# Nicholasli1995/SNVC

Measured on AMD Instinct MI355X. Metric: stereo-pairs/sec (cost-volume build + 3D CNN fwd), higher is better.
Workload: dtype f32 (split f16x3 operands, fp32 accumulate)

## Files before the change

snvc_amd/csrc/conv3d_f16.hip:

```cpp
#include <type_traits>

#include "common.hpp"
#include "elementwise_internal.hpp"
#include "snvc_fused.h"

namespace snvc {
namespace {

typedef _Float16 h8 __attribute__((ext_vector_type(8)));
typedef float f32x16 __attribute__((ext_vector_type(16)));
typedef float f32x4 __attribute__((ext_vector_type(4)));

__device__ const unsigned g_zero16h[4] __attribute__((aligned(16))) = {0u, 0u, 0u, 0u};

struct F16Args {
    const _Float16 *x;
    const _Float16 *wp;
    const float *scale, *bias;
    const _Float16 *res;
    _Float16 *y;
    float *y_f32;
    const _Float16 *x_lo, *res_lo;
    _Float16 *y_lo;
    const float *head;
    float *y_head;
    float head_mul;
    float res_mul;
    int *overflow;
    const _Float16 *tail_w;
    float *t_out;
    float tail_mul;
    int64_t t_bs;
    const float *res_f32;
    double *stats;
    const float *x_mul;
    int CGin;
    int Cout;
    int Din, Hin, Win;
    int Dout, Hout, Wout;
    int nd, nh, nw;
    int osd, osh, osw, offd, offh, offw;
    int pad_d, pad_h, pad_w;
    int isd, ish, iod, ioh;
    int tiles_d, tiles_h, tiles_w;
    int nchunks, flags;
    int N, cls_mode;
    int64_t cls_wstride;
    int64_t x_bs, y_bs, r_bs, yf_bs;
};

template <class I>
__host__ __device__ __forceinline__ I il_index(int mode, I oc, I C, I H, I pitch, I lp, I cls0, I h, I x) {
    const I cls = mode ? oc % 3 : oc / C, co = mode ? oc / 3 : oc % C, groups = (C + 7) / 8;
    return ((((cls0 + cls) * groups + (co >> 3)) * H + h) * pitch + lp + x) * 8 + (co & 7);
}

struct F16IlArgs : F16Args {
    float *y_il;
    int64_t il_bs;
    int il_mode, il_C, il_pitch, il_lp, il_cls0;
};

struct F16SrcArgs : F16Args {
    const float *gi;
    const float *p_il;
    const float *v_scale, *v_bias;
    int64_t gi_bs;
    int v_pitch, v_lp, v_q, v_m0, v_off, v_off2, v_flags;
};


template <int KD_, int KH_, int KW_, int STRIDE_, int DIL_, int MI_, int TD_, int TH_, int KCG_, int MODE_, bool DB_, int OCC_,
          int DILW_ = DIL_, int PL_ = 1, bool DYN_ = false>
struct F16Cfg {
    static constexpr bool DYN = DYN_;
    static constexpr int PL = PL_;
    static constexpr bool SPLIT = PL_ >= 2, SERIAL = PL_ == 3;
    static constexpr int RES_PL = PL_ == 2 ? 2 : 1;
    static constexpr int PASSES = SERIAL ? 2 : 1;
    static constexpr int PF = DYN_ ? 2 : (SPLIT ? 3 : 6);
    static constexpr int KD = KD_, KH = KH_, KW = KW_, STRIDE = STRIDE_, DIL = DIL_, DILW = DILW_, MI = MI_, TD = TD_, TH = TH_;
    static constexpr int KCG = KCG_, MODE = MODE_, OCC = OCC_;
    static constexpr bool DB = DB_;
    static constexpr int IN_D = (TD - 1) * STRIDE + (KD - 1) * DIL + 1;
    static constexpr int IN_H = (TH - 1) * STRIDE + (KH - 1) * DIL + 1;
    static constexpr int IN_W = 31 * STRIDE + (KW - 1) * DILW + 1;
    static constexpr int VOX = IN_D * IN_H * IN_W;
    static constexpr int GB = VOX * 16;
    static constexpr int ITEMS = RES_PL * KCG * VOX;
    static constexpr int PLANE_BYTES = KCG * GB;
    static constexpr int NIT = (ITEMS + 255) / 256;
    static constexpr int IMG_BYTES = NIT * 256 * 16;
    static constexpr int LDS_BYTES = IMG_BYTES * (DB ? 2 : 1);
    static constexpr int NB = TD * TH / 4;
    static constexpr bool UNROLL_D = KD <= 3;
    static constexpr int SEGS = UNROLL_D ? 1 : KD;
    static constexpr int TSEG = UNROLL_D ? KD * KH * KW : KH * KW;
    static constexpr int NPS = (TSEG + 1) / 2;
    static constexpr int NS = MODE == 0 ? TSEG * (KCG / 2) : NPS * KCG;
    static constexpr int STEPS = SEGS * NS;
    static constexpr int SEG_BYTES = DIL * IN_H * IN_W * 16;
    static_assert(TD * TH % 4 == 0, "rows split over 4 waves");
// ... 520 lines not shown
__device__ __forceinline__ void lds_read_b128_to(h8 &v, unsigned addr) {
    asm volatile("ds_read_b128 %0, %1 offset:%2" : "=v"(v) : "v"(addr), "n"(IMM) : "memory");
}

template <int N>
__device__ __forceinline__ void wait_lgkm_for(h8 (&b)[8]) {
    asm volatile("s_waitcnt lgkmcnt(%8)"
                 : "+v"(b[0]), "+v"(b[1]), "+v"(b[2]), "+v"(b[3]), "+v"(b[4]), "+v"(b[5]), "+v"(b[6]), "+v"(b[7])
                 : "n"(N)
                 : "memory");
}

template <int SRC, class A>
__device__ __forceinline__ const F16SrcArgs &src_args_of(const A &a) {
    if constexpr (SRC == 1) return a;
    else return *reinterpret_cast<const F16SrcArgs *>(&a);
}

template <int EPI, int SRC = 0>
__global__ void __launch_bounds__(256, 2)
conv3d_x3q_kernel(const std::conditional_t<SRC == 1, F16SrcArgs, F16Args> a) {
    using Cfg = X3QCfg;
    constexpr int NB = Cfg::NB, TH = Cfg::TH, IN_H = Cfg::IN_H, IN_W = Cfg::IN_W, VOX = Cfg::VOX, NIT = Cfg::NIT, NQ = Cfg::NQ;
    constexpr int ITEMS = Cfg::ITEMS, PF = Cfg::PF;
    extern __shared__ __attribute__((aligned(16))) char lds[];
    const int tid = threadIdx.x, lane = tid & 63, wave = tid >> 6, kb = lane >> 4, col = lane & 15;
    const int ntiles = a.tiles_d * a.tiles_h * a.tiles_w, cblocks = a.Cout >> 5;
    const int job = xcd_remap16(blockIdx.x, ntiles * cblocks);
    const int t = job / cblocks, cb = job - t * cblocks;
    const int tw = t % a.tiles_w, th = (t / a.tiles_w) % a.tiles_h, td = t / (a.tiles_w * a.tiles_h);
    const int64_t n = blockIdx.z;
    const int od0 = td * Cfg::TD, oh0 = th * TH, ow0 = tw * 32;
    const int id0 = od0 - a.pad_d, ih0 = oh0 - a.pad_h, iw0 = ow0 - a.pad_w;

    f32x4q acc[NB][2][2];
#pragma unroll
    for (int nb = 0; nb < NB; ++nb)
#pragma unroll
        for (int ph = 0; ph < 2; ++ph)
#pragma unroll
            for (int h = 0; h < 2; ++h) acc[nb][ph][h] = f32x4q{0.0f, 0.0f, 0.0f, 0.0f};

    const int in_hw = a.Hin * a.Win, in_dhw = in_hw * a.Din;
    unsigned off[NIT];
    unsigned vmask = 0, pmask = 0;
#pragma unroll
    for (int it = 0; it < NIT; ++it) {
        const int i = it * 256 + tid;
        const int plane = i / VOX, r = i - plane * VOX;
        pmask |= (unsigned)(plane & 1) << it;
        const int dd = r / (IN_H * IN_W), r2 = r - dd * (IN_H * IN_W);
        const int hh = r2 / IN_W, ww = r2 - hh * IN_W;
        const int gd = id0 + dd, gh = ih0 + hh, gw = iw0 + ww;
        const bool ok = i < ITEMS && (unsigned)gd < (unsigned)a.Din && (unsigned)gh < (unsigned)a.Hin && (unsigned)gw < (unsigned)a.Win;
        off[it] = ok ? (unsigned)(gd * in_hw + gh * a.Win + gw) : 0u;
        vmask |= (ok ? 1u : 0u) << it;
    }
    const _Float16 *xn = a.x + n * a.x_bs, *xn_lo = a.x_lo + n * a.x_bs;
    const int wbase = tid & ~63;
    auto issue = [&](int chunk, int buf) {
        const int64_t coff = (int64_t)chunk * in_dhw * 8;
        char *const ibuf = lds + buf * Cfg::IMG_BYTES;
#pragma unroll
        for (int it = 0; it < NIT; ++it) {
            const _Float16 *xc = (((pmask >> it) & 1u) ? xn_lo : xn) + coff;
            const void *src = ((vmask >> it) & 1u) ? static_cast<const void *>(xc + (size_t)off[it] * 8) : static_cast<const void *>(g_zero16h);
// ... 287 lines not shown
    for (int nb = 0; nb < NB; ++nb) {
        const int row = wave * NB + nb;
        const int pd = od0 + row / TH, phh = oh0 + row % TH;
#pragma unroll
        for (int ph = 0; ph < 2; ++ph) {
            const int pw = ow0 + 16 * ph + col;
            const bool ok = pd < a.nd && phh < a.nh && pw < a.nw;
            const int64_t sp = ok ? ((int64_t)pd * out_hw + phh * a.Wout + pw) : 0;
            h8 o, ol;
            float hsum = 0.0f;
#pragma unroll
            for (int e = 0; e < 8; ++e) {
                float v = __builtin_fmaf(acc[nb][ph][e >> 2][e & 3], sc[e], bi[e]);
                v = __builtin_amdgcn_fmed3f(v, lo_bound, kHalfMax);
                vmax = __builtin_fmaxf(vmax, ok ? __builtin_fabsf(v) : 0.0f);
                if constexpr (EPI == 3) hsum += hw8[e] * v;
                o[e] = (_Float16)v;
                ol[e] = (_Float16)(v - (float)o[e]);
            }
            if (ok) {
                *reinterpret_cast<h8 *>(yn + sp * 8) = o;
                *reinterpret_cast<h8 *>(yn_lo + sp * 8) = ol;
            }
            if constexpr (EPI == 3) {
                float tot = hsum + __shfl_xor(hsum, 16, 64);
                tot += __shfl_xor(tot, 32, 64);
                if (ok && kb == 0) a.y_head[n * out_dhw + sp] = tot * a.head_mul;
            }
        }
    }
    if (vmax >= kHalfMax && a.overflow) atomicOr(a.overflow, 1);
}

template <int KH_, int KW_>
struct X2QCfg {
    static constexpr int KH = KH_, KW = KW_, TH = 16, NB = 4, IN_H = TH + KH - 1, IN_W = 32 + KW - 1, VOX = IN_H * IN_W, GB = VOX * 16;
    static constexpr int ITEMS = 2 * VOX, PLANE_BYTES = GB, NIT = (ITEMS + 255) / 256;
    static constexpr int IMG_BYTES = NIT * 256 * 16, LDS_BYTES = 2 * IMG_BYTES;
    static constexpr int TAPS = KH * KW, NQ = (TAPS + 3) / 4, PF = 2, FILL_STEP = NQ - PF;
    static_assert(NQ > PF, "the refill is issued PF k-steps before the chunk ends");
};

template <class Cfg, int IL = 0>
__global__ void __launch_bounds__(256, 2)
conv2d_x3q_kernel(const std::conditional_t<IL == 1, F16IlArgs, F16Args> a) {
    constexpr int NB = Cfg::NB, IN_W = Cfg::IN_W, VOX = Cfg::VOX, NIT = Cfg::NIT, NQ = Cfg::NQ;
    constexpr int ITEMS = Cfg::ITEMS, PF = Cfg::PF;
    extern __shared__ __attribute__((aligned(16))) char lds[];
    const int tid = threadIdx.x, lane = tid & 63, wave = tid >> 6, kb = lane >> 4, col = lane & 15;
    const int ntiles = a.tiles_h * a.tiles_w, cblocks = a.Cout >> 5;
    const int job = xcd_remap16(blockIdx.x, ntiles * cblocks);
    const int t = job / cblocks, cb = job - t * cblocks;
    const int tw = t % a.tiles_w, th = t / a.tiles_w;
    const int64_t n = blockIdx.z;
    const int oh0 = th * Cfg::TH, ow0 = tw * 32;
    const int ih0 = oh0 - a.pad_h, iw0 = ow0 - a.pad_w;

    f32x4q acc[NB][2][2];
#pragma unroll
    for (int nb = 0; nb < NB; ++nb)
#pragma unroll
        for (int ph = 0; ph < 2; ++ph)
#pragma unroll
            for (int h = 0; h < 2; ++h) acc[nb][ph][h] = f32x4q{0.0f, 0.0f, 0.0f, 0.0f};

    const int in_hw = a.Hin * a.Win;
// ... 863 lines not shown

struct Q16Layout { int K3, NSEG, NQ, NH, NPL, PASSES; };

struct F16Form {
    PackArgs pack;
    Q16Layout q16;
    int MI, KCG;
    int chunk_frags;
    int pad_frags;
    int cls_mode, TD, TH, grid;
    bool split_res, stats;
    const char *unsupported;
    F16Launch launch[F16_CALLS];

    constexpr F16Form on(F16Call c, F16Launch l) const { F16Form f = *this; f.launch[c] = l; return f; }
};

template <class Cfg, int EPI>
void launch_f16(const F16Args &a, const F16Geom &g, hipStream_t st) {
    launch_lds<conv3d_f16_kernel<Cfg, EPI>>(g.grid, 256, Cfg::LDS_BYTES, st, a);
}
template <class Cfg>
void launch_q16s(const F16Args &a, const F16Geom &g, hipStream_t st) {
    launch_lds<conv3d_q16s_kernel<Cfg>>(g.grid, 256, Cfg::LDS_BYTES, st, a);
}
template <int EPI>
void launch_x3q(const F16Args &a, const F16Geom &g, hipStream_t st) {
    launch_lds<conv3d_x3q_kernel<EPI>>(g.grid, 256, X3QCfg::LDS_BYTES, st, a);
}
template <int EPI>
void launch_x3q_src(const F16Args &a, const F16Geom &g, hipStream_t st) {
    launch_lds<conv3d_x3q_kernel<EPI, 1>>(g.grid, 256, X3QCfg::LDS_BYTES, st, static_cast<const F16SrcArgs &>(a));
}
void launch_x3s2q(const F16Args &a, const F16Geom &g, hipStream_t st) {
    int wg = device_cu_count();
    if (wg <= 0) wg = 256;
    if (g.jobs < wg) wg = g.jobs >= 8 ? (int)(g.jobs & ~(int64_t)7) : (int)g.jobs;
    launch_lds<conv3d_x3s2q_kernel>(dim3((unsigned)wg), X3S2Cfg::THREADS, X3S2Cfg::LDS_BYTES, st, a, (int)g.jobs);
}

template <class Cfg, int... EPI>
constexpr F16Form f16_form(int cls_mode, bool stats = false) {
    constexpr F16Call call_of[5] = {TO_C8, TO_PLANE, TO_F32, TO_HEAD, TO_TAIL};
    constexpr int npl = Cfg::PL >= 2 ? 2 : 1;
    F16Form f{};
    f.pack.KD = Cfg::KD; f.pack.KH = Cfg::KH; f.pack.KW = Cfg::KW; f.pack.KCG = Cfg::KCG; f.pack.MODE = Cfg::MODE; f.pack.MI = Cfg::MI;
    f.pack.SEGS = Cfg::SEGS; f.pack.TSEG = Cfg::TSEG; f.pack.NPS = Cfg::NPS; f.pack.NS = Cfg::NS; f.pack.unroll_d = Cfg::UNROLL_D ? 1 : 0;
    f.pack.PL = Cfg::PL; f.pack.PASSES = Cfg::PASSES; f.pack.dyn = Cfg::DYN ? 1 : 0;
    f.MI = Cfg::MI; f.KCG = Cfg::KCG; f.TD = Cfg::TD; f.TH = Cfg::TH;
    f.chunk_frags = Cfg::PASSES * Cfg::STEPS * Cfg::MI * npl;
    f.pad_frags = Cfg::PF * Cfg::MI * npl;
    f.cls_mode = cls_mode; f.grid = GRID_TILES; f.split_res = true; f.stats = stats;
    f.unsupported = Cfg::PL >= 2 ? "snvc_f16x3_conv3d_forward: no kernel" : "snvc_f16_conv3d_forward: no kernel";
    ((f.launch[call_of[EPI]] = launch_f16<Cfg, EPI>), ...);
    return f;
}

constexpr F16Form q16_form(Q16Layout q, int TD, int TH, int pad_steps, int cls_mode, int grid, bool split_res, bool stats, const char *unsupported) {
    F16Form f{};
    f.q16 = q; f.MI = q.NH / 2; f.KCG = 1; f.TD = TD; f.TH = TH;
    f.chunk_frags = q.PASSES * q.NSEG * q.NQ * q.NH * q.NPL;
    f.pad_frags = pad_steps * q.NH * q.NPL;
    f.cls_mode = cls_mode; f.grid = grid; f.split_res = split_res; f.stats = stats; f.unsupported = unsupported;
    return f;
}
template <class C>
// ... 367 lines not shown
    a.res_f32 = c.res_f32;
    a.stats = c.stats;
    a.x_mul = to_f32 ? c.x_mul : nullptr;
    a.tail_w = reinterpret_cast<const _Float16 *>(c.tail_w); a.t_out = c.t_out; a.tail_mul = c.tail_mul;
    a.t_bs = (int64_t)27 * 8 * d->Din * d->Hin * d->Win;
    a.CGin = d->Cin / 8; a.Cout = d->Cout;
    a.Din = d->Din; a.Hin = d->Hin; a.Win = d->Win;
    a.Dout = d->Dout; a.Hout = d->Hout; a.Wout = d->Wout;
    a.nchunks = p.nchunks; a.flags = flags;
    a.x_bs = d->x_batch_stride ? d->x_batch_stride : 2 * (int64_t)d->Cin * in_sp;
    a.y_bs = d->y_batch_stride ? d->y_batch_stride : 2 * (int64_t)d->Cout * out_sp;
    a.r_bs = d->res_batch_stride ? d->res_batch_stride : 2 * (int64_t)d->Cout * out_sp;
    a.yf_bs = plane ? out_sp : (d->y_batch_stride ? d->y_batch_stride : (int64_t)d->Cout * out_sp);
    const F16Geom g = f16_geometry(*d, p, a);
    if (g.ntiles >= ((int64_t)1 << 30) || (int64_t)d->N * g.classes > 65535)
        return fail(SNVC_ERR_UNSUPPORTED, "snvc_f16x3_conv3d_forward: too many tiles or samples");
    hipStream_t st = as_stream(c.stream);
    if (c.stats_slots) {
        if (!(to_f32 && !plane && !tail && f.stats))
            return fail(SNVC_ERR_UNSUPPORTED, "snvc_f16x3_conv3d_forward_stats: this layer's kernel form has no statistics epilogue");
        *c.stats_slots = g.stats_slots;
        if (!c.stats) return fail(SNVC_ERR_INVALID_ARGUMENT, "snvc_f16x3_conv3d_forward_stats: null workspace");
        if (g.classes > 1) {
            const hipError_t e = hipMemsetAsync(c.stats, 0, (size_t)d->N * g.stats_slots * ((d->Cout + 31) / 32) * 64 * sizeof(double), st);
            if (e != hipSuccess) return fail(SNVC_ERR_HIP, "snvc_f16x3_conv3d_forward_stats: hipMemsetAsync failed");
        }
    }
    if (c.src && !f.launch[TO_SRC])
        return fail(SNVC_ERR_UNSUPPORTED, "snvc_fused_first_conv3d_forward: a 3x3x3 stride-1 layer on the 16x16x32 form (SNVC_ALGO_X3_Q16)");
    const F16Call call = tail ? TO_TAIL : plane ? TO_PLANE : to_f32 ? TO_F32 : c.head ? (c.src ? TO_SRC_HEAD : TO_HEAD) : (c.src ? TO_SRC : TO_C8);
    if (!f.launch[call] || (resflags && !f.split_res)) return fail(SNVC_ERR_UNSUPPORTED, f.unsupported);
    if (g.jobs >= ((int64_t)1 << 30)) return fail(SNVC_ERR_UNSUPPORTED, "snvc_f16x3_conv3d_forward: too many tiles");
    if (c.src && to_f32) return fail(SNVC_ERR_UNSUPPORTED, "snvc_fused_first_conv3d_forward: a split C8 output");
    f.launch[call](b, g, st);
    return check_launch("snvc_f16x3_conv3d_forward");
}

int snvc_f16x3_conv3d_forward(const snvc_conv3d_desc *d, const void *x_hi, const void *x_lo, const void *packed_weight,
                              const float *scale, const float *bias, const void *res_hi, const void *res_lo, void *y_hi,
                              void *y_lo, float *y_f32, const float *head, float *y_head, float head_mul, float res_mul,
                              int *overflow, void *stream) {
    F16x3Call c;
    c.x_hi = x_hi; c.x_lo = x_lo; c.packed_weight = packed_weight; c.scale = scale; c.bias = bias;
    c.res_hi = res_hi; c.res_lo = res_lo; c.y_hi = y_hi; c.y_lo = y_lo; c.y_f32 = y_f32;
    c.head = head; c.y_head = y_head; c.head_mul = head_mul; c.res_mul = res_mul; c.overflow = overflow; c.stream = stream;
    if (d && (d->flags & (SNVC_EPI_ADD_PRE | SNVC_EPI_ADD_POST)) == SNVC_EPI_ADD_POST && y_f32 && d->Cout != 1 && res_hi && !res_lo) {
        c.res_f32 = static_cast<const float *>(res_hi);
        c.res_hi = nullptr;
    }
    return f16x3_forward(d, c);
}

int snvc_fused_first_conv3d_forward(const snvc_conv3d_desc *d, const void *packed_weight, const float *scale, const float *bias, void *y_hi,
                                    void *y_lo, const float *head, float *y_head, float head_mul, int *overflow, const float *gi,
                                    int64_t pitch, int64_t lp, const float *p_il, const float *v_scale, const float *v_bias, int q, int m0,
                                    int off, int off2, int v_flags, void *stream) {
    using namespace snvc;
    if (!d || !gi || !p_il || !v_scale || !v_bias) return fail(SNVC_ERR_INVALID_ARGUMENT, "snvc_fused_first_conv3d_forward: null pointer");
    if (d->transposed || d->ksize != 3 || d->stride != 1 || d->pad != 1 || d->dilation != 1 || d->Cin % 8 || d->Din < 1 || d->Hin < 1 || d->Win < 1 ||
        (q != 1 && q != 2) || (v_flags & ~SNVC_EPI_RELU))
        return fail(SNVC_ERR_UNSUPPORTED, "snvc_fused_first_conv3d_forward: a 3x3x3 / stride 1 / pad 1 layer, Cin % 8 == 0, q = 1 | 2");
    if ((reinterpret_cast<uintptr_t>(gi) | reinterpret_cast<uintptr_t>(p_il) | reinterpret_cast<uintptr_t>(v_scale) | reinterpret_cast<uintptr_t>(v_bias)) & 31)
        return fail(SNVC_ERR_INVALID_ARGUMENT, "snvc_fused_first_conv3d_forward: gi / p_il / v_scale / v_bias must be 32-byte aligned");
    const int64_t D = d->Din, H = d->Hin, W = d->Win, CG = d->Cin / 8;
    const int64_t lo_g = -(D - 1) - m0 + off, hi_g = (int64_t)q * (W - 2) - m0 + off;
    const int64_t lo_c = (int64_t)q * (W - 1) - (D - 1) - m0 + off2, hi_c = (int64_t)q * (W - 1) - m0 + off2;
    if (lp < 0 || pitch <= 0 || lp + lo_c < 0 || lp + hi_c >= pitch || (W > 1 && (lp + lo_g < 0 || lp + hi_g >= pitch)))
        return fail(SNVC_ERR_INVALID_ARGUMENT, "snvc_fused_first_conv3d_forward: pitch / lp do not cover the G indices of this shape");
    if (6 * CG * H * pitch * 32 >= ((int64_t)1 << 31) || 3 * CG * H * W * 32 >= ((int64_t)1 << 31))
        return fail(SNVC_ERR_UNSUPPORTED, "snvc_fused_first_conv3d_forward: one sample of gi / p_il must stay below 2 GiB");
    F16SrcArgs s{};
    s.gi = gi; s.p_il = p_il; s.v_scale = v_scale; s.v_bias = v_bias; s.gi_bs = 6 * CG * H * pitch * 8;
    s.v_pitch = (int)pitch; s.v_lp = (int)lp; s.v_q = q; s.v_m0 = m0; s.v_off = off; s.v_off2 = off2; s.v_flags = v_flags;
    F16x3Call c;
    c.packed_weight = packed_weight; c.scale = scale; c.bias = bias; c.y_hi = y_hi; c.y_lo = y_lo;
    c.head = head; c.y_head = y_head; c.head_mul = head_mul; c.res_mul = 1.0f; c.overflow = overflow; c.src = &s; c.stream = stream;
    return f16x3_forward(d, c);
}

int64_t snvc_f16x3_conv3d_stats_workspace_bytes(const snvc_conv3d_desc *d) {
    using namespace snvc;
    F16Plan p;
    if (!d || d->N < 0 || make_f16_plan(*d, p, true)) return -1;
    const int64_t groups = (d->Cout + 31) / 32;
    F16Args a{};
    const int64_t slots = f16_geometry(*d, p, a).stats_slots;
    return (d->N * slots * groups * 64 + conv_stats_fold_scratch_doubles(d->N, (int)groups, slots) + d->N * (int64_t)d->Cout * 2) * (int64_t)sizeof(double);
}

int snvc_f16x3_conv3d_forward_f32(const snvc_conv3d_desc *d, const void *x_hi, const void *x_lo, const void *packed_weight,
                                  const float *scale, const float *bias, const float *x_mul, const float *res_f32, float *y_f32,
                                  float out_mul, void *stream) {
    using namespace snvc;
    if (!d || !y_f32) return fail(SNVC_ERR_INVALID_ARGUMENT, "snvc_f16x3_conv3d_forward_f32: null pointer");
    if (d->flags & (SNVC_EPI_ADD_PRE | SNVC_EPI_ADD_POST)) return fail(SNVC_ERR_INVALID_ARGUMENT, "snvc_f16x3_conv3d_forward_f32: the residual is res_f32 (added after the activation), no flag");
    F16x3Call c;
    c.x_hi = x_hi; c.x_lo = x_lo; c.packed_weight = packed_weight; c.scale = scale; c.bias = bias; c.x_mul = x_mul;
    c.res_f32 = res_f32; c.y_f32 = y_f32; c.head_mul = out_mul; c.res_mul = 1.0f; c.stream = stream;
    return f16x3_forward(d, c);
}

int snvc_f16x3_conv3d_forward_stats(const snvc_conv3d_desc *d, const void *x_hi, const void *x_lo, const void *packed_weight,
                                    const float *scale, const float *bias, const float *x_mul, float *y_f32, float head_mul, const float *gamma,
                                    const float *beta, float *bn_scale, float *bn_shift, float *mean, float *var, void *workspace,
                                    float eps, void *stream) {
    using namespace snvc;
    if (!d || !y_f32 || !bn_scale || !bn_shift || !workspace)
        return fail(SNVC_ERR_INVALID_ARGUMENT, "snvc_f16x3_conv3d_forward_stats: null pointer");
    if (d->N <= 0 || d->flags || d->Cout % 32) return fail(SNVC_ERR_UNSUPPORTED, "snvc_f16x3_conv3d_forward_stats: whole 32-channel groups, no epilogue flags");
    double *stats = static_cast<double *>(workspace);
// ... 241 lines not shown
```

snvc_amd/models/stereo_volume.py:

```python
import dataclasses
import itertools
import warnings
import weakref

import torch
import torch.nn as nn

from ..extension.build_cost_volume import _BuildCostVolume, build_cost_volume
from .. import ops
from .._derived import derived, fresh, stamp
from .submodule import (_ROUTES, SCRATCH_ATTRS, WORKSPACE_ATTRS, X3_GROUP_NORM, ConvBNReLU3d, HipConv3d, SplitModePolicy, SplitOverflow,
                        SplitT, _FactoredFirstConvFn, _ShearedFirstConvBNFn, _ShearedFirstConvFn, _folded_bn,
                        _is_channel_head as _is_head_conv, _Plan, convbn_3d, folded_head_weights, hourglass, overflow_guard, plan_for,
                        sheared_geometry, sheared_kernels, x3_exponent, x3_norm_bound, EPI_RELU, SHEAR_CLASS_KDS)

_PREP_EPOCH = itertools.count(1)
_X3_KEY = {ops.Conv3dLayer: "", ops.Conv2dLayerX3: "_x3"}
_ASK = object()


@dataclasses.dataclass
class _Prep:
    plans: dict
    c: int
# ... 70 lines not shown

    def last_first_layer(self) -> torch.Tensor:
        ws = self.__dict__.get("_snvc_ws", {})
        which = self.__dict__.get("_snvc_last_v1", "v1")
        if which == "v1s_lazy":
            return ops.from_split(ws[("v1s_lazy", (), None)](), self.__dict__["_snvc_x3"]["exp"]["v1"])
        for k, v in ws.items():
            if k[0] == which == "v1s":
                st = self.__dict__.get("_snvc_x3")
                return ops.from_split(v, st["exp"]["v1"] if st is not None else
                                      x3_exponent(x3_norm_bound(self.conv1[0][1], plan_for(self.conv1[0][0], "_x3", v.device))))
            if k[0] == which:
                return v
        raise RuntimeError("no first-layer result in the workspace")

    def release_workspace(self):
        for name in WORKSPACE_ATTRS:
            self.__dict__.pop(name, None)

    def train(self, mode: bool = True):
        if mode:
            self.release_workspace()
        return super().train(mode)

    def __getstate__(self):
        state = self.__dict__.copy()
        for name in SCRATCH_ATTRS:
            state.pop(name, None)
        return state

    arithmetic = "auto"
    stream_out = False
    fused_first = True
    split_prep = True
    fused_tail = True

    def _x3_state(self, device):
        hg = self.hg_conv3d
        seqs = {"conv2": self.conv2[0], "h1": hg.conv1[0], "h2": hg.conv2, "h3": hg.conv3[0], "h4": hg.conv4[0], "h5": hg.conv5}
        c = self.conv2[0][0].out_channels
        if c != 32 or self.conv2[0][0].in_channels != 32 or not _is_head_conv(self.classifier, c):
            return None
        norms = [self.conv1[0][1]] + [sq[1] for sq in seqs.values()]
        for nm in norms:
            if not isinstance(nm, nn.BatchNorm3d) or nm.training or nm.running_mean is None:
                return None
        tensors = [t for sq in list(seqs.values()) + [hg.conv6] for t in (sq[0].weight, sq[1].weight, sq[1].bias, sq[1].running_mean, sq[1].running_var)]
        tensors.append(self.classifier.weight)
        tensors += [self.conv1[0][1].weight, self.conv1[0][1].bias, self.conv1[0][1].running_mean, self.conv1[0][1].running_var]
        st = self.__dict__.get("_snvc_x3")
        if st is not None and fresh(st["stamp"], tensors, (device,)):
            return st
        e = {k: x3_exponent(x3_norm_bound(sq[1], plan_for(sq[0], "_x3", device))) for k, sq in [("v1", self.conv1[0])] + list(seqs.items())}
        st = {"stamp": stamp(tensors, (device,)), "exp": e, "layers": {}, "affine": {}}
        geo = {"conv2": (1, False), "h1": (2, False), "h2": (1, False), "h3": (2, False), "h4": (1, False), "h5": (2, True)}
        for k, sq in seqs.items():
            w = sq[0].weight.detach().to(device)
            st["layers"][k] = ops.Conv3dLayerX3(w, 3, geo[k][0], 1, 1, geo[k][1])
            st["affine"][k] = _folded_bn(sq[1], plan_for(sq[0], "", device))
        w5 = hg.conv5[0].weight.detach().double().abs()
        sets = ([1], [0, 2])
        l1 = None
        for pd in range(2):
            for ph in range(2):
                for pw in range(2):
                    t = w5[:, :, sets[pd]][:, :, :, sets[ph]][:, :, :, :, sets[pw]].sum(dim=(0, 2, 3, 4))
# ... 12 lines not shown
        self.__dict__["_snvc_x3"] = st
        return st

    @staticmethod
    def _x3_v1_affine(st, scale, bias):
        e1 = st["exp"]["v1"]
        return derived(st, "v1_affine", (scale, bias), lambda: ((scale * 2.0 ** e1).contiguous(), (bias * 2.0 ** e1).contiguous()))

    def _x3_select(self, device, arithmetic=None):
        mode = arithmetic or self.arithmetic
        if mode == "fp32" or torch.is_grad_enabled() or self.training or self.split_off:
            if mode == "x3":
                raise RuntimeError("arithmetic='x3' needs inference (no autograd, eval mode) and no earlier overflow")
            return None
        st = self._x3_state(device)
        if st is None:
            if mode == "x3":
                raise RuntimeError("arithmetic='x3': the stack does not qualify (32 channels, eval-mode BatchNorm3d everywhere)")
            return None
        return st if self.split_guard(device, mode) is not None else None

    def _tail_x3(self, st, v1s, timing=None, fused=None):
        L, A, E, flag = st["layers"], st["affine"], st["exp"], st["flag"]
        if fused is not None:
            (n, _, d, h, w), dev = fused[0], fused[1]
        else:
            n, dev = v1s.size(0), v1s.device
            d, h, w = v1s.shape[3:6]
        hg = self.hg_conv3d
        _mark(timing, "conv2", 0)
        v2_out = self._buffer("v2s", (n, 2, 4, d, h, w, 8), dev, torch.float16)
        if fused is not None:
            v2s, hv = L["conv2"].forward_fused_first(n=n, in_sp=(d, h, w), x_exp=E["v1"], scale=A["conv2"][0], bias=A["conv2"][1], flags=EPI_RELU,
                                                     out_exp=E["conv2"], head=self.classifier.weight, overflow=flag, out=v2_out, **fused[2])
            _ROUTES["fused_first_conv"] += 1
        else:
            v2s, hv = L["conv2"](v1s, E["v1"], *A["conv2"], flags=EPI_RELU, out_exp=E["conv2"], head=self.classifier.weight, overflow=flag,
                                 out=v2_out)
        _mark(timing, "conv2", 1)
        _ROUTES["side_head"] += 1
        o = L["h1"](v2s, E["conv2"], *A["h1"], flags=EPI_RELU, out_exp=E["h1"], overflow=flag)
        pre = L["h2"](o, E["h1"], *A["h2"], flags=EPI_RELU, out_exp=E["h2"], overflow=flag)
        o = L["h3"](pre, E["h2"], *A["h3"], flags=EPI_RELU, out_exp=E["h3"], overflow=flag)
        o = L["h4"](o, E["h3"], *A["h4"], flags=EPI_RELU, out_exp=E["h4"], overflow=flag)
        st["guard"].post()
        if st["tail"] is not None and self.fused_tail:
            t = L["h5"].forward_tail(o, E["h4"], *A["h5"], st["tail"], residual=pre, res_exp=E["h2"], flags=EPI_RELU | ops.EPI_ADD_PRE,
                                     out_exp=E["post"], overflow=flag, out=self._buffer("tail_t", (n, 27, 8) + tuple(o.shape[3:6]), dev))
            cost = ops.deconv_tail_gather(t, st["tail_bias"], hv)
            _ROUTES["x3_fused_tail"] += 1
        else:
            post = L["h5"](o, E["h4"], *A["h5"], residual=pre, flags=EPI_RELU | ops.EPI_ADD_PRE, out_exp=E["h2"], to_f32=True)
            cost = hg.conv6.fused(post, residual=None, head=self.classifier, head_residual=hv)
        _ROUTES["x3_tail"] += 1
        if self.overflow_check == "call" and st["guard"].wait():
            raise SplitOverflow()
        return cost

    def _tail(self, v, hv=None):
        cost, _, _ = self.hg_conv3d(v, None, None, residual=v, head=self.classifier, head_residual=hv)
        return cost

    def _gn_qualifies(self, device, arithmetic=None):
        mode = arithmetic or self.arithmetic
        norms = [m for m in self.modules() if isinstance(m, (nn.GroupNorm, nn.modules.batchnorm._BatchNorm))]
        if (not norms or not all(isinstance(m, nn.GroupNorm) for m in norms) or not X3_GROUP_NORM[0] or mode == "fp32"
                or torch.is_grad_enabled() or self.training or self.split_off or device.type != "cuda"
# ... 517 lines not shown
```

snvc_amd/ops.py:

```python
import contextlib
import ctypes
import math
import threading
import time
from typing import Optional, Tuple

import torch

from . import _derived, _fused, _lib
from ._lib import (EPI_ADD_POST, EPI_ADD_PRE, EPI_RELU, EPI_SIGMOID, EPI_STREAM_OUT, F32, F64, Conv3dDesc,
                   Unsupported, check)

__all__ = [
    "cost_volume_forward", "cost_volume_forward_right", "cost_volume_backward", "cost_volume_backward_right", "depth_class_sums", "voxel_gather_forward", "voxel_gather_backward",
    "Conv3dLayer", "conv_variant", "conv3d_wgrad", "Conv3dLayerF16", "to_c8", "from_c8", "voxel_gather_forward_f16",
    "mul_broadcast_c8", "avgpool_depth4_c8", "volume_resample", "rect_to_psv_grid", "act_backward_reduce", "act_backward_apply", "bn_backward_coefs", "norm_stats", "affine_act", "mul_broadcast", "avgpool_depth4", "zero_stuff2x",
    "disparity_regression", "argmax_rows", "roiaware_pool3d_forward", "roiaware_pool3d_backward",
    "points_in_boxes_gpu", "points_in_boxes_cpu",
    "EPI_RELU", "EPI_ADD_PRE", "EPI_ADD_POST", "EPI_SIGMOID", "EPI_STREAM_OUT",
]


_variant_bits = 0


@contextlib.contextmanager
def conv_variant(algo_bits: int):
    global _variant_bits
    prev = _variant_bits
    _variant_bits = int(algo_bits)
    try:
        yield
    finally:
        _variant_bits = prev


def _algo(exact: bool = False) -> int:
    return (_variant_bits | _lib.ALGO_DIRECT) if exact else _variant_bits


def _gpu(t: torch.Tensor, name: str):
    if not t.is_cuda:
# ... 1360 lines not shown
    x = x.contiguous()
    if x.dtype != torch.float32 or x.dim() != 4:
        raise RuntimeError("conv2d_x3_from_f32 needs a float32 [N,C,H,W] tensor")
    n, c, h, w = x.shape
    key = (n, c, h, w, tuple(id(l) for l in layers), x.device)
    if ws.get("key") != key:
        ws.clear()
        ws.update(key=key, split=torch.empty(n * 2 * c * h * w, dtype=torch.float16, device=x.device),
                  mul=torch.empty(1, dtype=torch.float32, device=x.device),
                  y=[torch.empty((n, l.cout, h, w), dtype=torch.float32, device=x.device) for l in layers])
        k = len(layers)
        ws["c_packed"] = (ctypes.c_void_p * k)(*[l.packed.data_ptr() for l in layers])
        ws["c_cout"] = (ctypes.c_int64 * k)(*[l.cout for l in layers])
        ws["c_mul"] = (ctypes.c_float * k)(*[2.0 ** -l.w_exp for l in layers])
        ws["c_y"] = (ctypes.c_void_p * k)(*[t.data_ptr() for t in ws["y"]])
        ws["layers"] = list(layers)
    scratch = _scale_scratch(x.device)
    with torch.cuda.device(x.device):
        check(_lib.lib().snvc_f16x3_conv2d_from_f32(_ptr(x), n, c, h, w, layers[0].kh, layers[0].kw, len(layers), ws["c_packed"], ws["c_cout"],
                                                    ws["c_mul"], ws["c_y"], _ptr(ws["split"]), _ptr(scratch), _ptr(ws["mul"]), _stream(x)),
              "snvc_f16x3_conv2d_from_f32")
    return ws["y"]



def il_index(mode: int, oc: int, c: int, h_dim: int, pitch: int, lp: int, cls0: int, h: int, x: int) -> int:
    return int(_fused.lib().snvc_fused_il_index(mode, oc, c, h_dim, pitch, lp, cls0, h, x))


def fused_il_geometry(q: int, m0: int, d: int, w: int, wu: int, off: int, wu_col: int, off_col: int):
    lo = min(0, q * (w - 1) - (d - 1) - m0 + off_col, -(d - 1) - m0 + off if w > 1 else 0)
    hi = max(wu - 1, wu_col - 1, q * (w - 1) - m0 + off_col, q * (w - 2) - m0 + off if w > 1 else 0)
    return hi - lo + 1, -lo


def sheared_prep_x3_il(right, q: int, wu: int, off: int, wu_col: int, off_col: int, lay_g: "Conv2dLayerX3", lay_col: "Conv2dLayerX3", ws: dict,
                       pitch: int, lp: int):
    _gpu(right, "right")
    right = right.contiguous()
    n, c, h, w = right.shape
    key = (n, c, h, w, wu, wu_col, pitch, lp, right.device)
    if ws.get("key") != key:
        dev = right.device
        ws.clear()
        ws.update(key=key, rq=torch.empty(n * 2 * c * h * wu, dtype=torch.float16, device=dev),
                  rq2=torch.empty(n * 2 * c * h * wu_col, dtype=torch.float16, device=dev), mul=torch.empty(1, dtype=torch.float32, device=dev),
                  g=torch.empty((n, lay_g.cout, h, wu), dtype=torch.float32, device=dev),
                  gcol=torch.empty((n, lay_col.cout, h, wu_col), dtype=torch.float32, device=dev),
                  gi=torch.zeros((n, 6, c // 8, h, pitch, 8), dtype=torch.float32, device=dev))
    scratch = _scale_scratch(right.device)
    with torch.cuda.device(right.device):
        check(_fused.lib().snvc_fused_sheared_prep_x3(_ptr(right), n, c, h, w, int(q), int(wu), int(off), int(wu_col), int(off_col),
                                                      _ptr(lay_g.packed), _ptr(lay_col.packed), lay_g.cout, float(2.0 ** -lay_g.w_exp),
                                                      float(2.0 ** -lay_col.w_exp), _ptr(ws["rq"]), _ptr(ws["rq2"]), _ptr(scratch), _ptr(ws["mul"]),
                                                      _ptr(ws["g"]), _ptr(ws["gcol"]), _ptr(ws["gi"]), int(pitch), int(lp), _stream(right)),
              "snvc_fused_sheared_prep_x3")
    return ws["g"], ws["gcol"], ws["gi"]


def planes_x3_il(x, layer: "Conv2dLayerX3", ws: dict):
    _gpu(x, "x")
    x = x.contiguous()
    if x.dtype != torch.float32 or x.dim() != 4:
        raise RuntimeError("planes_x3_il needs a float32 [N,C,H,W] tensor")
    n, c, h, w = x.shape
    key = (n, c, h, w, id(layer), "il", x.device)
# ... 156 lines not shown
        if self.w_mul_dev is not None and scale is None and bias is None and x_exp == 0 and out_exp == 0:
            sc, bi = self._unit_affine(x.device)
            if x_mul_dev is not None:
                sc = sc / x_mul_dev
        else:
            sc, bi = self.folded(scale, bias, x_exp, out_exp)
            if x_mul_dev is not None:
                sc = (sc / x_mul_dev).contiguous()
            if self.w_mul_dev is not None:
                sc = (sc / self.w_mul_dev).contiguous()
        if n == 0:
            return out_f32 if f32 else ((out, y_head) if head is not None else out)
        d = self._desc(n, in_sp, flags, algo, _batch_stride(x), _batch_stride(out_f32 if f32 else out),
                       _batch_stride(residual) if residual is not None else 0)
        null = ctypes.c_void_p(0)
        with torch.cuda.device(x.device):
            check(_lib.lib().snvc_f16x3_conv3d_forward(ctypes.byref(d), _ptr(x), _lo_ptr(x), _ptr(packed), _ptr(sc), _ptr(bi),
                                                       _ptr(residual if residual_f32 is None else residual_f32),
                                                       _lo_ptr(residual) if residual is not None else null,
                                                       null if f32 else _ptr(out), null if f32 else _lo_ptr(out),
                                                       _ptr(out_f32) if f32 else null, _ptr(head), _ptr(y_head), float(2.0 ** -out_exp),
                                                       float(2.0 ** (out_exp - (out_exp if res_exp is None else res_exp))),
                                                       _ptr(overflow), _stream(x)), "snvc_f16x3_conv3d_forward")
        if f32:
            return out_f32
        return (out, y_head) if head is not None else out

    def fused_first_form(self, n: int, sp) -> bool:
        return (self.ksize == 3 and self.stride == 1 and not self.transposed and self.w_mul_dev is None and self.cin % 8 == 0
                and x3_form(self.cout, 3, 1, self.dilation, False, n, tuple(sp), True, False, self.forced_algo) == _lib.ALGO_X3_Q16)

    def forward_fused_first(self, gi, pitch: int, lp: int, p_il, v_scale, v_bias, q: int, m0: int, off: int, off_col: int, v_flags: int,
                            n: int, in_sp, x_exp: int = 0, scale=None, bias=None, flags: int = 0, out=None, out_exp: int = 0, head=None,
                            overflow=None):
        in_sp = tuple(int(v) for v in in_sp)
        if not self.fused_first_form(n, in_sp):
            raise Unsupported("forward_fused_first: the layer does not run on the 16x16x32 form at this size")
        algo = self.algo = _lib.ALGO_X3_Q16
        packed = self._pack(algo)
        out_sp = self.out_spatial(in_sp)
        out = _result(out, (n, 2, self.cout // 8) + out_sp + (8,), torch.float16, gi.device,
                      "conv3d `out` must be a split C8 tensor of the output shape", _split_check)
        y_head = None
        if head is not None:
            head = head.detach().reshape(-1).float().contiguous()
            y_head = torch.empty((n, 1) + out_sp, dtype=torch.float32, device=gi.device)
        sc, bi = self.folded(scale, bias, x_exp, out_exp)
        if n == 0:
            return (out, y_head) if head is not None else out
        d = self._desc(n, in_sp, flags, algo, 0, _batch_stride(out), 0)
        with torch.cuda.device(gi.device):
            check(_fused.lib().snvc_fused_first_conv3d_forward(ctypes.byref(d), _ptr(packed), _ptr(sc), _ptr(bi), _ptr(out), _lo_ptr(out),
                                                               _ptr(head), _ptr(y_head), float(2.0 ** -out_exp), _ptr(overflow), _ptr(gi),
                                                               int(pitch), int(lp), _ptr(p_il), _ptr(v_scale), _ptr(v_bias), int(q), int(m0),
                                                               int(off), int(off_col), int(v_flags), _stream(gi)),
                  "snvc_fused_first_conv3d_forward")
        return (out, y_head) if head is not None else out

    def forward_f32(self, x, x_mul_dev, residual_f32: Optional[torch.Tensor] = None, relu: bool = False):
        _split_check(x, "x")
        if self.w_mul_dev is None or x.size(2) * 8 != self.cin:
            raise RuntimeError("forward_f32: a device-scaled layer (w_mul_dev) and an input of its channel count")
        n, in_sp, out_sp, algo, packed = self._launch(x, plain=True, split_out=False)
        sc, bi = self._unit_affine(x.device)
        y = torch.empty((n, self.cout) + out_sp, dtype=torch.float32, device=x.device)
        if residual_f32 is not None:
            _residual_f32_check(residual_f32, y)
        if n == 0:
            return y
        d = self._desc(n, in_sp, EPI_RELU if relu else 0, algo, _batch_stride(x), _batch_stride(y), 0)
        with torch.cuda.device(x.device):
            check(_lib.lib().snvc_f16x3_conv3d_forward_f32(ctypes.byref(d), _ptr(x), _lo_ptr(x), _ptr(packed), _ptr(sc), _ptr(bi),
                                                           _ptr(x_mul_dev), _ptr(residual_f32), _ptr(y), 1.0, _stream(x)),
                  "snvc_f16x3_conv3d_forward_f32")
        return y

    def forward_stats(self, x, x_mul_dev, gamma, beta, eps: float):
        _split_check(x, "x")
        if self.w_mul_dev is None or x.size(2) * 8 != self.cin or self.cout % 32:
            return None
        n, in_sp, out_sp, algo, packed = self._launch(x, plain=True, split_out=False)
        sc, bi = self._unit_affine(x.device)
        raw = torch.empty((n, self.cout) + out_sp, dtype=torch.float32, device=x.device)
        d = self._desc(n, in_sp, 0, algo, _batch_stride(x), _batch_stride(raw), 0)
        nbytes = _lib.lib().snvc_f16x3_conv3d_stats_workspace_bytes(ctypes.byref(d))
        if nbytes < 0:
            return None
        ws = torch.empty(nbytes, dtype=torch.uint8, device=x.device)
        out = torch.empty((4, self.cout), dtype=torch.float32, device=x.device)
# ... 192 lines not shown
```

Baseline: 536.5.

## Skip duplicate wedge tiles in fused first conv and replicate outputs by copy

Adds a dedup path for the fused cost-volume + first 3D conv. Output tiles inside the pure wedge region, where the sheared volume is constant along disparity, have inputs identical to the tile above. Those tiles return early, and a follow-up copy kernel replicates a representative tile's output (hi/lo planes and head) into them. This removes redundant MMA work at the cost of an extra launch and copy traffic, and it depends on the wedge predicate being exact.

```diff
diff --git a/include/snvc_dedup.h b/include/snvc_dedup.h
--- /dev/null
+++ b/include/snvc_dedup.h
@@ -0,0 +1,26 @@
+#ifndef SNVC_DEDUP_H
+#define SNVC_DEDUP_H
+
+#include <stdint.h>
+
+#include "snvc_hip.h"
+
+#ifdef __cplusplus
+extern "C" {
+#endif
+
+SNVC_API int snvc_dedup_abi_version(void);
+
+SNVC_API int snvc_dedup_fused_first_conv3d_forward(const snvc_conv3d_desc *desc, const void *packed_weight, const float *scale,
+                                                   const float *bias, void *y_hi, void *y_lo, const float *head, float *y_head,
+                                                   float head_mul, int *overflow, const float *gi, int64_t pitch, int64_t lp,
+                                                   const float *p_il, const float *v_scale, const float *v_bias, int q, int m0, int off,
+                                                   int off2, int v_flags, void *stream);
+
+SNVC_API int64_t snvc_dedup_fused_first_tiles(const snvc_conv3d_desc *desc, int q, int m0, int off, int64_t *first_td, int64_t *last_td,
+                                              int max_tw);
+
+#ifdef __cplusplus
+}
+#endif
+#endif
diff --git a/snvc_amd/_dedup.py b/snvc_amd/_dedup.py
--- /dev/null
+++ b/snvc_amd/_dedup.py
@@ -0,0 +1,31 @@
+import ctypes
+
+from . import _fused, _lib
+
+_ABI = 1
+
+c_i64 = ctypes.c_int64
+c_int = ctypes.c_int
+
+SIGNATURES = {
+    "snvc_dedup_abi_version": (c_int, []),
+    "snvc_dedup_fused_first_conv3d_forward": _fused.SIGNATURES["snvc_fused_first_conv3d_forward"],
+    "snvc_dedup_fused_first_tiles": (c_i64, [ctypes.POINTER(_lib.Conv3dDesc), c_int, c_int, c_int, ctypes.POINTER(c_i64),
+                                             ctypes.POINTER(c_i64), c_int]),
+}
+
+_bound = None
+
+
+def lib() -> ctypes.CDLL:
+    global _bound
+    if _bound is None:
+        handle = _lib.lib()
+        for name, (res, args) in SIGNATURES.items():
+            fn = getattr(handle, name)
+            fn.restype = res
+            fn.argtypes = args
+        if handle.snvc_dedup_abi_version() != _ABI:
+            raise RuntimeError("libsnvc_hip.so wedge deduplication ABI version mismatch; rebuild it")
+        _bound = handle
+    return _bound
diff --git a/snvc_amd/csrc/conv3d_f16.hip b/snvc_amd/csrc/conv3d_f16.hip
--- a/snvc_amd/csrc/conv3d_f16.hip
+++ b/snvc_amd/csrc/conv3d_f16.hip
@@ -3,6 +3,7 @@
 #include "common.hpp"
 #include "elementwise_internal.hpp"
 #include "snvc_fused.h"
+#include "snvc_dedup.h"
 
 namespace snvc {
 namespace {
@@ -68,6 +69,14 @@
     int64_t gi_bs;
     int v_pitch, v_lp, v_q, v_m0, v_off, v_off2, v_flags;
 };
+constexpr int SRC_DEDUP = 1 << 30;
+
+__host__ __device__ __forceinline__ bool wedge_tile_pure(int D, int W, int q, int m0, int off, int d0, int w0) {
+    return d0 >= 2 && d0 + 3 <= D - 3 && w0 + 32 < W - 1 && q * (w0 + 32) - (d0 - 1) - m0 + off < 0;
+}
+__host__ __device__ __forceinline__ bool wedge_tile_duplicate(int D, int W, int q, int m0, int off, int d0, int w0) {
+    return wedge_tile_pure(D, W, q, m0, off, d0, w0) && wedge_tile_pure(D, W, q, m0, off, d0 - 4, w0);
+}
 
 
 template <int KD_, int KH_, int KW_, int STRIDE_, int DIL_, int MI_, int TD_, int TH_, int KCG_, int MODE_, bool DB_, int OCC_,
@@ -654,6 +663,9 @@
     const int64_t n = blockIdx.z;
     const int od0 = td * Cfg::TD, oh0 = th * TH, ow0 = tw * 32;
     const int id0 = od0 - a.pad_d, ih0 = oh0 - a.pad_h, iw0 = ow0 - a.pad_w;
+    if constexpr (SRC == 1) {
+        if ((a.v_flags & SRC_DEDUP) && wedge_tile_duplicate(a.Din, a.Win, a.v_q, a.v_m0, a.v_off, od0, ow0)) return;
+    }
 
     f32x4q acc[NB][2][2];
 #pragma unroll
@@ -1007,6 +1019,57 @@
     if (vmax >= kHalfMax && a.overflow) atomicOr(a.overflow, 1);
 }
 
+struct WedgeCopyArgs {
+    _Float16 *y, *y_lo;
+    float *y_head;
+    int64_t y_bs;
+    int CG, D, H, W, q, m0, off;
+    int td0, ntw;
+};
+
+__global__ void __launch_bounds__(256)
+wedge_copy_kernel(const WedgeCopyArgs a) {
+    const int tw = blockIdx.x % a.ntw, td = a.td0 + blockIdx.x / a.ntw;
+    const int d0 = td * X3QCfg::TD, w0 = tw * 32, h0 = blockIdx.y * X3QCfg::TH;
+    if (!wedge_tile_duplicate(a.D, a.W, a.q, a.m0, a.off, d0, w0)) return;
+    int rep = d0 - X3QCfg::TD;
+    while (wedge_tile_pure(a.D, a.W, a.q, a.m0, a.off, rep - X3QCfg::TD, w0)) rep -= X3QCfg::TD;
+    const int64_t n = blockIdx.z, hw = (int64_t)a.H * a.W, dhw = hw * a.D;
+    const int tid = threadIdx.x;
+    const int col = tid & 31, h = h0 + ((tid >> 5) & 3);
+    const int rounds = 2 * a.CG * 128 / 256;
+    if (h < a.H) {
+        for (int r0 = 0; r0 < rounds; r0 += 4) {
+            uint4 *p[4];
+            uint4 v[4];
+#pragma unroll
+            for (int k = 0; k < 4; ++k) {
+                const int g = 2 * (r0 + k) + (tid >> 7);
+                const bool on = r0 + k < rounds;
+                const int plane = on ? g / a.CG : 0, cg = on ? g - plane * a.CG : 0;
+                p[k] = reinterpret_cast<uint4 *>((plane ? a.y_lo : a.y) + n * a.y_bs) + (cg * dhw + (int64_t)h * a.W + w0 + col);
+                if (on) v[k] = p[k][rep * hw];
+            }
+#pragma unroll
+            for (int k = 0; k < 4; ++k) {
+                if (r0 + k < rounds) {
+#pragma unroll
+                    for (int r = 0; r < X3QCfg::TD; ++r) p[k][(d0 + r) * hw] = v[k];
+                }
+            }
+        }
+    }
+    if (a.y_head && tid < 32) {
+        const int hh = h0 + (tid >> 3);
+        if (hh < a.H) {
+            uint4 *p = reinterpret_cast<uint4 *>(a.y_head + n * dhw + (int64_t)hh * a.W + w0) + (tid & 7);
+            const uint4 v = p[rep * hw / 4];
+#pragma unroll
+            for (int r = 0; r < X3QCfg::TD; ++r) p[(d0 + r) * hw / 4] = v;
+        }
+    }
+}
+
 template <int KH_, int KW_>
 struct X2QCfg {
     static constexpr int KH = KH_, KW = KW_, TH = 16, NB = 4, IN_H = TH + KH - 1, IN_W = 32 + KW - 1, VOX = IN_H * IN_W, GB = VOX * 16;
@@ -1936,6 +1999,33 @@
 void launch_x3q_src(const F16Args &a, const F16Geom &g, hipStream_t st) {
     launch_lds<conv3d_x3q_kernel<EPI, 1>>(g.grid, 256, X3QCfg::LDS_BYTES, st, static_cast<const F16SrcArgs &>(a));
 }
+struct WedgeRange { int64_t dups; int td0, td1, ntw; };
+WedgeRange wedge_ranges(int D, int W, int q, int m0, int off, int64_t *first_td, int64_t *last_td, int max_tw) {
+    WedgeRange r{0, -1, -1, 0};
+    const int tiles_d = (D + X3QCfg::TD - 1) / X3QCfg::TD, tiles_w = (W + 31) / 32;
+    for (int tw = 0; tw < tiles_w; ++tw) {
+        int first = -1, last = -1;
+        for (int td = 0; td < tiles_d; ++td) {
+            if (!wedge_tile_pure(D, W, q, m0, off, td * X3QCfg::TD, tw * 32)) continue;
+            if (first < 0) first = td;
+            last = td;
+        }
+        if (last == first) first = last = -1;
+        if (tw < max_tw && first_td && last_td) { first_td[tw] = first; last_td[tw] = last; }
+        if (first < 0) continue;
+        r.dups += last - first;
+        r.ntw = tw + 1;
+        if (tw == 0) { r.td0 = first + 1; r.td1 = last; }
+    }
+    return r;
+}
+void launch_wedge_copy(const F16SrcArgs &a, hipStream_t st) {
+    const WedgeRange r = wedge_ranges(a.Din, a.Win, a.v_q, a.v_m0, a.v_off, nullptr, nullptr, 0);
+    if (r.dups == 0) return;
+    WedgeCopyArgs w{a.y, a.y_lo, a.y_head, a.y_bs, a.Cout / 8, a.Dout, a.Hout, a.Wout, a.v_q, a.v_m0, a.v_off, r.td0, r.ntw};
+    wedge_copy_kernel<<<dim3((unsigned)((r.td1 - r.td0 + 1) * r.ntw), (unsigned)a.tiles_h, (unsigned)a.N), 256, 0, st>>>(w);
+}
+
 void launch_x3s2q(const F16Args &a, const F16Geom &g, hipStream_t st) {
     int wg = device_cu_count();
     if (wg <= 0) wg = 256;
@@ -2369,7 +2459,11 @@
     if (!f.launch[call] || (resflags && !f.split_res)) return fail(SNVC_ERR_UNSUPPORTED, f.unsupported);
     if (g.jobs >= ((int64_t)1 << 30)) return fail(SNVC_ERR_UNSUPPORTED, "snvc_f16x3_conv3d_forward: too many tiles");
     if (c.src && to_f32) return fail(SNVC_ERR_UNSUPPORTED, "snvc_fused_first_conv3d_forward: a split C8 output");
+    if ((b.v_flags & SRC_DEDUP) && ((c.y_head && (d->Wout % 4 || (reinterpret_cast<uintptr_t>(c.y_head) & 15))) ||
+                                    wedge_ranges(a.Din, a.Win, b.v_q, b.v_m0, b.v_off, nullptr, nullptr, 0).dups == 0))
+        b.v_flags &= ~SRC_DEDUP;
     f.launch[call](b, g, st);
+    if (b.v_flags & SRC_DEDUP) launch_wedge_copy(b, st);
     return check_launch("snvc_f16x3_conv3d_forward");
 }
 
@@ -2388,10 +2482,10 @@
     return f16x3_forward(d, c);
 }
 
-int snvc_fused_first_conv3d_forward(const snvc_conv3d_desc *d, const void *packed_weight, const float *scale, const float *bias, void *y_hi,
-                                    void *y_lo, const float *head, float *y_head, float head_mul, int *overflow, const float *gi,
-                                    int64_t pitch, int64_t lp, const float *p_il, const float *v_scale, const float *v_bias, int q, int m0,
-                                    int off, int off2, int v_flags, void *stream) {
+static int fused_first_forward(const snvc_conv3d_desc *d, const void *packed_weight, const float *scale, const float *bias, void *y_hi,
+                               void *y_lo, const float *head, float *y_head, float head_mul, int *overflow, const float *gi,
+                               int64_t pitch, int64_t lp, const float *p_il, const float *v_scale, const float *v_bias, int q, int m0,
+                               int off, int off2, int v_flags, bool dedup, void *stream) {
     using namespace snvc;
     if (!d || !gi || !p_il || !v_scale || !v_bias) return fail(SNVC_ERR_INVALID_ARGUMENT, "snvc_fused_first_conv3d_forward: null pointer");
     if (d->transposed || d->ksize != 3 || d->stride != 1 || d->pad != 1 || d->dilation != 1 || d->Cin % 8 || d->Din < 1 || d->Hin < 1 || d->Win < 1 ||
@@ -2408,11 +2502,40 @@
         return fail(SNVC_ERR_UNSUPPORTED, "snvc_fused_first_conv3d_forward: one sample of gi / p_il must stay below 2 GiB");
     F16SrcArgs s{};
     s.gi = gi; s.p_il = p_il; s.v_scale = v_scale; s.v_bias = v_bias; s.gi_bs = 6 * CG * H * pitch * 8;
-    s.v_pitch = (int)pitch; s.v_lp = (int)lp; s.v_q = q; s.v_m0 = m0; s.v_off = off; s.v_off2 = off2; s.v_flags = v_flags;
+    s.v_pitch = (int)pitch; s.v_lp = (int)lp; s.v_q = q; s.v_m0 = m0; s.v_off = off; s.v_off2 = off2;
+    s.v_flags = v_flags | (dedup ? SRC_DEDUP : 0);
     F16x3Call c;
     c.packed_weight = packed_weight; c.scale = scale; c.bias = bias; c.y_hi = y_hi; c.y_lo = y_lo;
     c.head = head; c.y_head = y_head; c.head_mul = head_mul; c.res_mul = 1.0f; c.overflow = overflow; c.src = &s; c.stream = stream;
     return f16x3_forward(d, c);
+}
+
+int snvc_fused_first_conv3d_forward(const snvc_conv3d_desc *d, const void *packed_weight, const float *scale, const float *bias, void *y_hi,
+                                    void *y_lo, const float *head, float *y_head, float head_mul, int *overflow, const float *gi,
+                                    int64_t pitch, int64_t lp, const float *p_il, const float *v_scale, const float *v_bias, int q, int m0,
+                                    int off, int off2, int v_flags, void *stream) {
+    return fused_first_forward(d, packed_weight, scale, bias, y_hi, y_lo, head, y_head, head_mul, overflow, gi, pitch, lp, p_il, v_scale, v_bias,
+                               q, m0, off, off2, v_flags, false, stream);
+}
+
+int snvc_dedup_abi_version(void) { return 1; }
+
+int snvc_dedup_fused_first_conv3d_forward(const snvc_conv3d_desc *d, const void *packed_weight, const float *scale, const float *bias,
+                                          void *y_hi, void *y_lo, const float *head, float *y_head, float head_mul, int *overflow,
+                                          const float *gi, int64_t pitch, int64_t lp, const float *p_il, const float *v_scale,
+                                          const float *v_bias, int q, int m0, int off, int off2, int v_flags, void *stream) {
+    return fused_first_forward(d, packed_weight, scale, bias, y_hi, y_lo, head, y_head, head_mul, overflow, gi, pitch, lp, p_il, v_scale, v_bias,
+                               q, m0, off, off2, v_flags, true, stream);
+}
+
+int64_t snvc_dedup_fused_first_tiles(const snvc_conv3d_desc *d, int q, int m0, int off, int64_t *first_td, int64_t *last_td, int max_tw) {
+    using namespace snvc;
+    if (!d || d->Din < 1 || d->Win < 1 || (q != 1 && q != 2) || max_tw < 0 || (max_tw > 0 && (!first_td || !last_td))) {
+        fail(SNVC_ERR_INVALID_ARGUMENT, "snvc_dedup_fused_first_tiles: a desc, q = 1 | 2, and max_tw entries to write");
+        return -1;
+    }
+    for (int tw = 0; tw < max_tw; ++tw) first_td[tw] = last_td[tw] = -1;
+    return wedge_ranges((int)d->Din, (int)d->Win, q, m0, off, first_td, last_td, max_tw).dups;
 }
 
 int64_t snvc_f16x3_conv3d_stats_workspace_bytes(const snvc_conv3d_desc *d) {
diff --git a/snvc_amd/models/stereo_volume.py b/snvc_amd/models/stereo_volume.py
--- a/snvc_amd/models/stereo_volume.py
+++ b/snvc_amd/models/stereo_volume.py
@@ -126,6 +126,7 @@
     arithmetic = "auto"
     stream_out = False
     fused_first = True
+    dedup_wedge = True
     split_prep = True
     fused_tail = True
 
@@ -204,7 +205,8 @@
         v2_out = self._buffer("v2s", (n, 2, 4, d, h, w, 8), dev, torch.float16)
         if fused is not None:
             v2s, hv = L["conv2"].forward_fused_first(n=n, in_sp=(d, h, w), x_exp=E["v1"], scale=A["conv2"][0], bias=A["conv2"][1], flags=EPI_RELU,
-                                                     out_exp=E["conv2"], head=self.classifier.weight, overflow=flag, out=v2_out, **fused[2])
+                                                     out_exp=E["conv2"], head=self.classifier.weight, overflow=flag, out=v2_out,
+                                                     dedup=bool(self.dedup_wedge), **fused[2])
             _ROUTES["fused_first_conv"] += 1
         else:
             v2s, hv = L["conv2"](v1s, E["v1"], *A["conv2"], flags=EPI_RELU, out_exp=E["conv2"], head=self.classifier.weight, overflow=flag,
diff --git a/snvc_amd/ops.py b/snvc_amd/ops.py
--- a/snvc_amd/ops.py
+++ b/snvc_amd/ops.py
@@ -7,7 +7,7 @@
 
 import torch
 
-from . import _derived, _fused, _lib
+from . import _dedup, _derived, _fused, _lib
 from ._lib import (EPI_ADD_POST, EPI_ADD_PRE, EPI_RELU, EPI_SIGMOID, EPI_STREAM_OUT, F32, F64, Conv3dDesc,
                    Unsupported, check)
 
@@ -1434,6 +1434,17 @@
     lo = min(0, q * (w - 1) - (d - 1) - m0 + off_col, -(d - 1) - m0 + off if w > 1 else 0)
     hi = max(wu - 1, wu_col - 1, q * (w - 1) - m0 + off_col, q * (w - 2) - m0 + off if w > 1 else 0)
     return hi - lo + 1, -lo
+
+
+def fused_first_wedge_tiles(d: int, w: int, q: int, m0: int, off: int):
+    desc = _lib.Conv3dDesc()
+    desc.Din, desc.Win = int(d), int(w)
+    ntw = (int(w) + 31) // 32
+    first, last = (ctypes.c_int64 * ntw)(), (ctypes.c_int64 * ntw)()
+    dups = int(_dedup.lib().snvc_dedup_fused_first_tiles(ctypes.byref(desc), int(q), int(m0), int(off), first, last, ntw))
+    if dups < 0:
+        raise ValueError(_lib.lib().snvc_last_error_string().decode())
+    return dups, list(first), list(last)
 
 
 def sheared_prep_x3_il(right, q: int, wu: int, off: int, wu_col: int, off_col: int, lay_g: "Conv2dLayerX3", lay_col: "Conv2dLayerX3", ws: dict,
@@ -1656,7 +1667,7 @@
 
     def forward_fused_first(self, gi, pitch: int, lp: int, p_il, v_scale, v_bias, q: int, m0: int, off: int, off_col: int, v_flags: int,
                             n: int, in_sp, x_exp: int = 0, scale=None, bias=None, flags: int = 0, out=None, out_exp: int = 0, head=None,
-                            overflow=None):
+                            overflow=None, dedup: bool = False):
         in_sp = tuple(int(v) for v in in_sp)
         if not self.fused_first_form(n, in_sp):
             raise Unsupported("forward_fused_first: the layer does not run on the 16x16x32 form at this size")
@@ -1673,12 +1684,12 @@
         if n == 0:
             return (out, y_head) if head is not None else out
         d = self._desc(n, in_sp, flags, algo, 0, _batch_stride(out), 0)
+        entry = (_dedup.lib().snvc_dedup_fused_first_conv3d_forward if dedup else _fused.lib().snvc_fused_first_conv3d_forward)
         with torch.cuda.device(gi.device):
-            check(_fused.lib().snvc_fused_first_conv3d_forward(ctypes.byref(d), _ptr(packed), _ptr(sc), _ptr(bi), _ptr(out), _lo_ptr(out),
-                                                               _ptr(head), _ptr(y_head), float(2.0 ** -out_exp), _ptr(overflow), _ptr(gi),
-                                                               int(pitch), int(lp), _ptr(p_il), _ptr(v_scale), _ptr(v_bias), int(q), int(m0),
-                                                               int(off), int(off_col), int(v_flags), _stream(gi)),
-                  "snvc_fused_first_conv3d_forward")
+            check(entry(ctypes.byref(d), _ptr(packed), _ptr(sc), _ptr(bi), _ptr(out), _lo_ptr(out), _ptr(head), _ptr(y_head),
+                        float(2.0 ** -out_exp), _ptr(overflow), _ptr(gi), int(pitch), int(lp), _ptr(p_il), _ptr(v_scale), _ptr(v_bias), int(q),
+                        int(m0), int(off), int(off_col), int(v_flags), _stream(gi)),
+                  "snvc_dedup_fused_first_conv3d_forward" if dedup else "snvc_fused_first_conv3d_forward")
         return (out, y_head) if head is not None else out
 
     def forward_f32(self, x, x_mul_dev, residual_f32: Optional[torch.Tensor] = None, relu: bool = False):
```

New measurement: 546.4, median of 6. +1.8%, better.
